# vkit-dev/vkit-ocr-model-adaptive-scaling

Hardware: AMD Instinct MI355X
Metric: images/sec fwd+bwd @1024x1024 bf16 (train step: rough+precise passes, losses, backward, clip, AdamW) (higher is better)
Workload: dtype bf16

## Files before the change

include/vkas.h:

```cpp
#ifndef VKAS_H
#define VKAS_H

#include <stddef.h>
#include <stdint.h>

#ifdef __cplusplus
extern "C" {
#endif

#define VKAS_F32 0
#define VKAS_BF16 1
#define VKAS_F16 2

#define VKAS_OK 0
#define VKAS_E_ARG (-1)
#define VKAS_E_LAUNCH (-2)

#define VKAS_EPI_NONE 0
#define VKAS_EPI_GELU 1
#define VKAS_EPI_SCALE_RES 2
#define VKAS_EPI_DGELU 3
#define VKAS_EPI_ADD 4
#define VKAS_EPI_PATCH 5
#define VKAS_EPI_HEAD 6
// ... 115 lines not shown
size_t vkas_layernorm_bwd_ws_bytes(long M, int Cp);

int vkas_pack_head_params(const float* gamma, const float* beta, const float* wproj, const float* bproj, int C, int oc,
                          int pw, float* out, void* stream);
int vkas_head_tail_fwd(const void* z, long ldz, const vkas_head_desc* hd, long M, int dtype, void* stream);
int vkas_head_tail_bwd(const void* z, long ldz, const vkas_head_desc* hd, const float* const* dproj, void* dz, long lddz,
                       float* dparams, float* ws, size_t ws_bytes, long M, int dtype, void* stream);
size_t vkas_head_tail_bwd_ws_bytes(long M, int pw);

int vkas_scale_res_bwd(const void* dout, long lddo, const void* z, long ldz, const float* colscale,
                       const float* rowscale, int rows_per_image, void* dz, long lddz, float* dscale, float* dbias,
                       float* ws, size_t ws_bytes, long M, int Cp, int dtype, void* stream);
size_t vkas_scale_res_bwd_ws_bytes(long M, int Cp);

int vkas_resize_fwd(const void* x, long ldx, void* y, long ldy, int B, int Hin, int Win, int Hout, int Wout,
                    int Cp, int mode, int accumulate, int dtype, void* stream);
int vkas_resize_bwd(const void* dy, long lddy, void* dx, long lddx, int B, int Hin, int Win, int Hout, int Wout,
                    int Cp, int mode, int accumulate, int dtype, void* stream);
size_t vkas_resize_bwd_ws_bytes(int B, int Hin, int Win, int Hout, int Wout, int Cp);
int vkas_resize_bwd_ws(const void* dy, long lddy, void* dx, long lddx, float* ws, size_t ws_bytes, int B, int Hin, int Win,
                       int Hout, int Wout, int Cp, int mode, int accumulate, int dtype, void* stream);

int vkas_upconv_adj(const void* dz, long lddz, void* E, int B, int h, int w, int N, int dtype, void* stream);
int vkas_upconv_adj_unpack_wgrad(const float* gE, float* gwp, int N, int Cp, void* stream);

int vkas_adaptive_avgpool_fwd(const void* x, long ldx, void* y, long ldy, int B, int H, int W, int s, int Cp,
                              int dtype, void* stream);
int vkas_adaptive_avgpool_bwd(const void* dy, long lddy, void* dx, long lddx, int B, int H, int W, int s, int Cp,
                              int accumulate, int dtype, void* stream);

int vkas_copy_channels(const void* x, long ldx, void* y, long ldy, long M, int Cp, int accumulate, int dtype,
                       void* stream);
int vkas_copy_channel_range(const void* x, long ldx, int c_src, void* y, long ldy, int c_dst, long M, int C,
                            int zero_tail, int dtype, void* stream);
int vkas_softplus_fwd(const float* x, float* y, long n, void* stream);
int vkas_softplus_bwd(const float* x, const float* dy, float* dx, long n, void* stream);

typedef struct vkas_rough_loss_cfg {
  float focal_factor, dice_factor, l1_factor, score_min, height_min;
  float focal_alpha, focal_gamma;
  float out_scale;
} vkas_rough_loss_cfg;
int vkas_rough_loss_fwd(const float* mask_feat, const float* height_feat, const float* gt_mask,
                        const float* gt_score, int B, int H, int W, int up, int left, int CH, int CW,
                        const vkas_rough_loss_cfg* cfg, double* sums, float* loss, void* stream);
int vkas_rough_loss_bwd(const float* mask_feat, const float* height_feat, const float* gt_mask,
// ... 42 lines not shown
#define VKAS_LOSS_FOCAL 0
#define VKAS_LOSS_DICE 1
#define VKAS_LOSS_L1 2
#define VKAS_LOSS_SMOOTH_L1 3
#define VKAS_LOSS_L2 4
#define VKAS_LOSS_WAHR 5
int vkas_elementwise_loss_fwd(int kind, const float* pred, const float* gt, const float* mask, long n, float p0, float p1,
                              float eps, double* sums, float* loss, void* stream);
int vkas_elementwise_loss_bwd(int kind, const float* pred, const float* gt, const float* mask, long n, float p0, float p1,
                              float eps, const double* sums, const float* dloss, float* dpred, void* stream);
int vkas_cross_entropy_fwd(const float* logits, const void* target, int hard, long rows, int classes, double* sums,
                           float* loss, void* stream);
int vkas_cross_entropy_bwd(const float* logits, const void* target, int hard, long rows, int classes, const float* dloss,
                           float* dlogits, void* stream);

int vkas_points_prepare(const long* py, const long* px, int B, int P, int H, int W, int* map, int* pix, long Mp, void* stream);
int vkas_points_gather_rows(const void* z, long ldz, int c0, int Ns, const float* stats, const float* const* dproj,
                            int n_heads, long M, const int* pix, long Mp, void* zs, float* stats_s, float* dproj_s,
                            int dtype, void* stream);
int vkas_points_gather_patches(const void* x, long ldx, int Cp, int B, int H, int W, const int* pix, long Mp, void* xs,
                               int dtype, void* stream);
int vkas_points_scatter3x3(const float* D, const int* pix, const int* map, long Mp, int B, int H, int W, int Cp, void* dx,
                           long lddx, int dtype, void* stream);

int vkas_points_scatter_vec8(const float* src, const int* pix, long Mp, float* dst, void* stream);
int vkas_points_gather_vec8(const float* src, const int* pix, long Mp, float* dst, void* stream);

typedef struct {
  const float* w;
  void* out;
  long total;
  int kind, N, C, KH, KW, Np, Cp, mode, n_off, Nt, dtype;
} vkas_pack_desc;
int vkas_pack_many(const vkas_pack_desc* descs, const int* block_start, int count, int total_blocks, void* stream);
int vkas_pack_many_blocks(const vkas_pack_desc* d);

int vkas_rough_postprocess(const float* mask_logit, const float* height, int B, int H, int W, const int* valid_h,
                           const int* valid_w, float mask_thr, float height_min, unsigned char* out_mask,
                           float* out_height, void* stream);
int vkas_precise_postprocess(const float* prob_logit, const float* offset, const float* angle, const float* dist, int B,
                             int H, int W, const int* valid_h, const int* valid_w, float* out_prob, float* out_offset,
                             float* out_angle, float* out_dist, void* stream);
long vkas_char_polygons_workspace_bytes(int B, int H, int W, int size);
int vkas_char_polygons(const float* prob, const float* offset, const float* angle, const float* dist, int B, int H, int W,
                       int size, float thr, float scale_y, float scale_x, void* workspace, size_t workspace_bytes,
                       int* count, int* points, float* probs, float* quads, void* stream);
// ... 20 lines not shown
```

vkit_ocr_model_adaptive_scaling_amd/_lib.py:

```python
import ctypes
import os
from ctypes import POINTER, Structure, c_char, c_char_p, c_double, c_float, c_int, c_int64, c_long, c_longlong, c_size_t, c_uint, c_void_p

_HERE = os.path.dirname(os.path.abspath(__file__))
LIB_PATH = os.environ.get('VKAS_LIB_PATH') or os.path.join(_HERE, 'libvkas.so')

F32, BF16, F16 = 0, 1, 2
EPI_NONE, EPI_GELU, EPI_SCALE_RES, EPI_DGELU, EPI_ADD, EPI_PATCH, EPI_HEAD = range(7)
LOSS_FOCAL, LOSS_DICE, LOSS_L1, LOSS_SMOOTH_L1, LOSS_L2 = range(5)
LOSS_WAHR = 5
PRECISE_LOSS_EX_SUMS = 16


class ConvGeom(Structure):
    _fields_ = [('B', c_int), ('Hin', c_int), ('Win', c_int), ('Hout', c_int), ('Wout', c_int), ('Cp', c_int),
                ('ldx', c_int), ('KH', c_int), ('KW', c_int), ('stride', c_int), ('pad', c_int)]


class HeadDesc(Structure):
    _fields_ = [('n_heads', c_int), ('pw', c_int), ('n0', c_int * 4), ('np', c_int * 4), ('c', c_int * 4),
                ('oc', c_int * 4), ('params', c_void_p), ('stats', c_void_p), ('proj', c_void_p)]


class Epilogue(Structure):
# ... 94 lines not shown
                                    POINTER(GemmPlanInfo)]),
    'vkas_colsum': (c_int, [_P, c_long, c_long, c_int, _P, c_int, _P, c_size_t, c_int, _P]),
    'vkas_colsum_ws_bytes': (c_size_t, [c_long, c_int]),
    'vkas_dwconv7x7_fwd': (c_int, [_P, c_long, _P, _P, _P, c_long, _P, c_long, c_int, c_int, c_int, c_int, c_int, _P]),
    'vkas_dwconv7x7_wgrad': (c_int, [_P, c_long, _P, c_long, _P, _P, _P, c_size_t, c_int, c_int, c_int, c_int, c_int, _P]),
    'vkas_dwconv7x7_wgrad_ws_bytes': (c_size_t, [c_int, c_int, c_int, c_int]),
    'vkas_layernorm_fwd': (c_int, [_P, c_long, _P, _P, _P, c_long, _P, c_long, c_int, c_int, c_int, c_int, _P]),
    'vkas_layernorm_bwd': (c_int, [_P, c_long, _P, _P, _P, _P, c_long, _P, c_long, _P, _P, _P, c_size_t, c_long, c_int,
                                   c_int, c_int, c_int, _P]),
    'vkas_layernorm_bwd_ws_bytes': (c_size_t, [c_long, c_int]),
    'vkas_pack_head_params': (c_int, [_P, _P, _P, _P, c_int, c_int, c_int, _P, _P]),
    'vkas_head_tail_fwd': (c_int, [_P, c_long, _P, c_long, c_int, _P]),
    'vkas_head_tail_bwd': (c_int, [_P, c_long, POINTER(HeadDesc), POINTER(c_void_p), _P, c_long, _P, _P, c_size_t, c_long, c_int, _P]),
    'vkas_head_tail_bwd_ws_bytes': (c_size_t, [c_long, c_int]),
    'vkas_scale_res_bwd': (c_int, [_P, c_long, _P, c_long, _P, _P, c_int, _P, c_long, _P, _P, _P, c_size_t, c_long,
                                   c_int, c_int, _P]),
    'vkas_scale_res_bwd_ws_bytes': (c_size_t, [c_long, c_int]),
    'vkas_resize_fwd': (c_int, [_P, c_long, _P, c_long, c_int, c_int, c_int, c_int, c_int, c_int, c_int, c_int, c_int, _P]),
    'vkas_resize_bwd': (c_int, [_P, c_long, _P, c_long, c_int, c_int, c_int, c_int, c_int, c_int, c_int, c_int, c_int, _P]),
    'vkas_resize_bwd_ws_bytes': (c_size_t, [c_int, c_int, c_int, c_int, c_int, c_int]),
    'vkas_resize_bwd_ws': (c_int, [_P, c_long, _P, c_long, _P, c_size_t, c_int, c_int, c_int, c_int, c_int, c_int, c_int, c_int,
                                   c_int, _P]),
    'vkas_upconv_adj': (c_int, [_P, c_long, _P, c_int, c_int, c_int, c_int, c_int, _P]),
    'vkas_upconv_adj_unpack_wgrad': (c_int, [_P, _P, c_int, c_int, _P]),
    'vkas_adaptive_avgpool_fwd':(c_int, [_P, c_long, _P, c_long, c_int, c_int, c_int, c_int, c_int, c_int, _P]),
    'vkas_adaptive_avgpool_bwd': (c_int, [_P, c_long, _P, c_long, c_int, c_int, c_int, c_int, c_int, c_int, c_int, _P]),
    'vkas_copy_channels': (c_int, [_P, c_long, _P, c_long, c_long, c_int, c_int, c_int, _P]),
    'vkas_copy_channel_range': (c_int, [_P, c_long, c_int, _P, c_long, c_int, c_long, c_int, c_int, c_int, _P]),
    'vkas_softplus_fwd': (c_int, [_P, _P, c_long, _P]),
    'vkas_softplus_bwd': (c_int, [_P, _P, _P, c_long, _P]),
    'vkas_rough_loss_fwd': (c_int, [_P, _P, _P, _P, c_int, c_int, c_int, c_int, c_int, c_int, c_int,
                                    POINTER(RoughLossCfg), _P, _P, _P]),
    'vkas_rough_loss_bwd': (c_int, [_P, _P, _P, _P, c_int, c_int, c_int, c_int, c_int, c_int, c_int,
                                    POINTER(RoughLossCfg), _P, _P, _P, _P, _P]),
    'vkas_points_margin': (c_int, [_P, _P, c_long, c_int, c_int, _P, _P]),
    'vkas_precise_loss_fwd': (c_int, [_P] * 11 + [c_int] * 8 + [POINTER(PreciseLossCfg), _P, _P, _P]),
    'vkas_precise_loss_bwd': (c_int, [_P] * 11 + [c_int] * 8 + [POINTER(PreciseLossCfg), _P, _P, _P, _P, _P, _P, _P]),
    'vkas_precise_loss_ex_fwd': (c_int, [_P] * 11 + [c_int] * 8 + [POINTER(PreciseLossCfg), _P, POINTER(PreciseLossExtraCfg),
                                                                     _P, _P, _P]),
    'vkas_precise_loss_ex_bwd': (c_int, [_P] * 11 + [c_int] * 8 + [POINTER(PreciseLossCfg), _P, POINTER(PreciseLossExtraCfg)]
                                 + [_P] * 8),
    'vkas_elementwise_loss_fwd': (c_int, [c_int, _P, _P, _P, c_long, c_float, c_float, c_float, _P, _P, _P]),
    'vkas_elementwise_loss_bwd': (c_int, [c_int, _P, _P, _P, c_long, c_float, c_float, c_float, _P, _P, _P, _P]),
    'vkas_cross_entropy_fwd': (c_int, [_P, _P, c_int, c_long, c_int, _P, _P, _P]),
    'vkas_cross_entropy_bwd': (c_int, [_P, _P, c_int, c_long, c_int, _P, _P, _P]),
    'vkas_points_prepare': (c_int, [_P, _P, c_int, c_int, c_int, c_int, _P, _P, c_long, _P]),
    'vkas_points_gather_rows': (c_int, [_P, c_long, c_int, c_int, _P, _P, c_int, c_long, _P, c_long, _P, _P, _P, c_int, _P]),
    'vkas_points_gather_patches': (c_int, [_P, c_long, c_int, c_int, c_int, c_int, _P, c_long, _P, c_int, _P]),
    'vkas_points_scatter3x3': (c_int, [_P, _P, _P, c_long, c_int, c_int, c_int, c_int, _P, c_long, c_int, _P]),
    'vkas_points_scatter_vec8': (c_int, [_P, _P, c_long, _P, _P]),
    'vkas_points_gather_vec8': (c_int, [_P, _P, c_long, _P, _P]),
    'vkas_pack_many': (c_int, [_P, _P, c_int, c_int, _P]),
    'vkas_pack_many_blocks': (c_int, [_P]),
    'vkas_rough_postprocess': (c_int, [_P, _P, c_int, c_int, c_int, _P, _P, c_float, c_float, _P, _P, _P]),
    'vkas_precise_postprocess': (c_int, [_P, _P, _P, _P, c_int, c_int, c_int, _P, _P, _P, _P, _P, _P, _P]),
    'vkas_char_polygons_workspace_bytes': (c_long, [c_int, c_int, c_int, c_int]),
    'vkas_char_polygons': (c_int, [_P, _P, _P, _P, c_int, c_int, c_int, c_int, c_float, c_float, c_float, _P, c_size_t,
                                   _P, _P, _P, _P, _P]),
    'vkas_text_regions_workspace_bytes': (c_longlong, [c_int, c_int, c_int, c_int]),
    'vkas_text_regions': (c_int, [_P, _P, c_int, c_int, c_int, c_int, _P, c_longlong, _P, _P, _P, _P, _P, _P, _P]),
    'vkas_resample_pack_u8': (c_int, [_P, c_int, c_int, _P, c_int, _P, c_int, c_int, _P]),
    'vkas_pack_region_labels': (c_int, [_P, c_int, c_int, c_int, c_int, c_int, c_int, _P, _P, c_int, c_int, _P, c_int, c_int,
                                        _P]),
    'vkas_l2norm_sq': (c_int, [_P, c_long, _P, _P]),
    'vkas_adamw_step': (c_int, [_P, _P, _P, _P, c_long, _P, c_float, c_float, c_float, c_float, c_float, c_float,
                                c_float, c_int, _P]),
}

EXPORTS = tuple(_SIGS)

for _name, (_res, _args) in _SIGS.items():
    _fn = getattr(lib, _name)
# ... 9 lines not shown
```

vkit_ocr_model_adaptive_scaling_amd/csrc/points.hip:

```cpp
#include "vkas_common.h"

namespace {

constexpr int PT_EMPTY = 0x7f7f7f7f;
constexpr int PT_PAD = INT_MIN;

__device__ __forceinline__ long pt_clamp(long v, int n) { return v < 0 ? 0 : (v > n - 1 ? n - 1 : v); }

__global__ __launch_bounds__(256) void points_claim_kernel(const long* __restrict__ py, const long* __restrict__ px, int P,
                                                           int H, int W, long n, int* __restrict__ map) {
  const long i = (long)blockIdx.x * 256 + threadIdx.x;
  if (i >= n) return;
  const long q = (i / P) * H * W + pt_clamp(py[i], H) * W + pt_clamp(px[i], W);
  atomicMin(&map[q], (int)i);
}

__global__ __launch_bounds__(256) void points_pix_kernel(const long* __restrict__ py, const long* __restrict__ px, int P, int H,
                                                         int W, long n, long Mp, const int* __restrict__ map,
                                                         int* __restrict__ pix) {
  const long i = (long)blockIdx.x * 256 + threadIdx.x;
  if (i >= Mp) return;
  if (i >= n) {
    pix[i] = PT_PAD;
    return;
// ... 78 lines not shown
    src[u] = o;
    if (o != PT_EMPTY && first) {
      first = false;
      mine = (o == (int)i && u == t);
    }
  }
  if (!mine) return;
  T* out = dx + (img + (long)ty * W + tx) * lddx;
  for (int v = threadIdx.x; v < (Cp >> 3); v += 64) {
    float acc[8];
    load8(out + v * 8, acc);
#pragma unroll
    for (int u = 0; u < 9; ++u) {
      if (src[u] == PT_EMPTY) continue;
      const float4* r = reinterpret_cast<const float4*>(D + ((long)src[u] * 9 + u) * Cp + v * 8);
      const float4 r0 = r[0], r1 = r[1];
      acc[0] += r0.x; acc[1] += r0.y; acc[2] += r0.z; acc[3] += r0.w;
      acc[4] += r1.x; acc[5] += r1.y; acc[6] += r1.z; acc[7] += r1.w;
    }
    store8(out + v * 8, acc);
  }
}

__global__ __launch_bounds__(256) void points_scatter_vec8_kernel(const float* __restrict__ src, const int* __restrict__ pix,
                                                                  long Mp, float* __restrict__ dst) {
  const long t = (long)blockIdx.x * 256 + threadIdx.x;
  const long i = t >> 1;
  if (i >= Mp) return;
  const int p = pix[i];
  if (p < 0) return;
  reinterpret_cast<float4*>(dst + (long)p * 8)[t & 1] = reinterpret_cast<const float4*>(src + i * 8)[t & 1];
}

__global__ __launch_bounds__(256) void points_gather_vec8_kernel(const float* __restrict__ src, const int* __restrict__ pix,
                                                                 long Mp, float* __restrict__ dst) {
  const long t = (long)blockIdx.x * 256 + threadIdx.x;
  const long i = t >> 1;
  if (i >= Mp) return;
  const int p = pix[i];
  float4 v = make_float4(0.f, 0.f, 0.f, 0.f);
  if (p >= 0) v = reinterpret_cast<const float4*>(src + (long)p * 8)[t & 1];
  reinterpret_cast<float4*>(dst + i * 8)[t & 1] = v;
}

}

// ... 58 lines not shown
                 vkas_aligned16(xs),
             "vkas_points_gather_patches: bad sizes Cp=%d ldx=%ld", Cp, ldx);
  hipStream_t st = vkas_stream(stream);
  VKAS_DISPATCH_DTYPE(dtype, "vkas_points_gather_patches", {
    points_gather_patches_kernel<T><<<(unsigned)Mp, 64, 0, st>>>((const T*)x, ldx, Cp, H, W, pix, (T*)xs);
  })
  VKAS_LAUNCH_CHECK("points_gather_patches");
  return VKAS_OK;
}

extern "C" int vkas_points_scatter3x3(const float* D, const int* pix, const int* map, long Mp, int B, int H, int W, int Cp,
                                      void* dx, long lddx, int dtype, void* stream) {
  VKAS_CHECK(D && pix && map && dx, "vkas_points_scatter3x3: null pointer");
  VKAS_CHECK(Cp > 0 && Cp % 8 == 0 && lddx >= Cp && lddx % 8 == 0 && B > 0 && H > 0 && W > 0 && Mp > 0 && Mp * 9 < 0x7fffffffL &&
                 vkas_aligned16(D) && vkas_aligned16(dx),
             "vkas_points_scatter3x3: bad sizes Cp=%d lddx=%ld Mp=%ld", Cp, lddx, Mp);
  hipStream_t st = vkas_stream(stream);
  VKAS_DISPATCH_DTYPE(dtype, "vkas_points_scatter3x3", {
    points_scatter3x3_kernel<T><<<(unsigned)(Mp * 9), 64, 0, st>>>(D, pix, map, H, W, Cp, (T*)dx, lddx);
  })
  VKAS_LAUNCH_CHECK("points_scatter3x3");
  return VKAS_OK;
}
```

vkit_ocr_model_adaptive_scaling_amd/csrc/upconv_adj.hip:

```cpp
#include "vkas_common.h"

namespace {

__device__ __forceinline__ int xcd_row(unsigned bx, unsigned rows) {
  const unsigned xcd = bx & 7u, slot = bx >> 3;
  const unsigned q8 = rows >> 3, r8 = rows & 7u;
  return (int)((xcd < r8 ? xcd * (q8 + 1) : r8 * (q8 + 1) + (xcd - r8) * q8) + slot);
}

__device__ __forceinline__ void ut_weights(int i, int n, float* w) {
  w[0] = i == 0 ? 0.f : 0.25f;
  w[1] = i == 0 ? 1.f : 0.75f;
  w[2] = i == n - 1 ? 1.f : 0.75f;
  w[3] = i == n - 1 ? 0.f : 0.25f;
}

template <typename T>
__global__ __launch_bounds__(256) void upconv_adj_kernel(const T* __restrict__ dz, long lddz, T* __restrict__ E, int h,
                                                         int w, int nvec) {
  const int idx = blockIdx.y * 256 + threadIdx.x;
  const int j = idx / nvec;
  const int v = idx - j * nvec;
  if (j >= w) return;
  const int row = xcd_row(blockIdx.x, gridDim.x);
  const int b = row / h;
  const int i = row - b * h;
  const int H2 = 2 * h, W2 = 2 * w;
  float wy[4], wx[4];
  ut_weights(i, h, wy);
  ut_weights(j, w, wx);
  int xc[6];
  bool xok[6];
#pragma unroll
  for (int c = 0; c < 6; ++c) {
    const int X = 2 * j - 2 + c;
    xok[c] = X >= 0 && X < W2;
    xc[c] = X < 0 ? 0 : (X >= W2 ? W2 - 1 : X);
  }
  const T* db = dz + (long)b * H2 * W2 * lddz + v * 8;
  float acc[3][3][8];
#pragma unroll
  for (int ky = 0; ky < 3; ++ky)
#pragma unroll
    for (int kx = 0; kx < 3; ++kx)
#pragma unroll
      for (int k = 0; k < 8; ++k) acc[ky][kx][k] = 0.f;
#pragma unroll
  for (int r = 0; r < 6; ++r) {
    const int Y = 2 * i - 2 + r;
    const bool yok = Y >= 0 && Y < H2;
    const int yc = Y < 0 ? 0 : (Y >= H2 ? H2 - 1 : Y);
    const T* rowp = db + (long)yc * W2 * lddz;
    Raw8<T> raw[6];
#pragma unroll
    for (int c = 0; c < 6; ++c) raw[c].load(rowp + (long)xc[c] * lddz);
    float hs[3][8];
#pragma unroll
    for (int kx = 0; kx < 3; ++kx)
#pragma unroll
      for (int k = 0; k < 8; ++k) hs[kx][k] = 0.f;
#pragma unroll
    for (int c = 0; c < 6; ++c) {
      raw[c].keep_if(yok && xok[c]);
      float t[8];
      raw[c].unpack(t);
#pragma unroll
      for (int kx = 0; kx < 3; ++kx) {
        const int a = c - kx;
        if (a < 0 || a > 3) continue;
#pragma unroll
        for (int k = 0; k < 8; ++k) hs[kx][k] = fmaf(wx[a], t[k], hs[kx][k]);
      }
    }
#pragma unroll
    for (int ky = 0; ky < 3; ++ky) {
      const int a = r - ky;
      if (a < 0 || a > 3) continue;
#pragma unroll
      for (int kx = 0; kx < 3; ++kx)
#pragma unroll
        for (int k = 0; k < 8; ++k) acc[ky][kx][k] = fmaf(wy[a], hs[kx][k], acc[ky][kx][k]);
    }
  }
  const long N = (long)nvec * 8;
  T* dst = E + (((long)b * h + i) * w + j) * (9 * N) + v * 8;
#pragma unroll
  for (int ky = 0; ky < 3; ++ky)
#pragma unroll
    for (int kx = 0; kx < 3; ++kx) store8(dst + (ky * 3 + kx) * N, acc[ky][kx]);
}

__global__ __launch_bounds__(256) void upconv_adj_unpack_kernel(const float* __restrict__ gE, float* __restrict__ gwp, int N,
                                                                int Cp4, long total4) {
  for (long i = (long)blockIdx.x * 256 + threadIdx.x; i < total4; i += (long)gridDim.x * 256) {
    const int c4 = (int)(i % Cp4);
    const long r = i / Cp4;
    const int n = (int)(r % N);
    const int k = (int)(r / N);
    const float4 s = reinterpret_cast<const float4*>(gE)[i];
    float4* d = reinterpret_cast<float4*>(gwp) + ((long)n * 9 + (8 - k)) * Cp4 + c4;
    float4 o = *d;
    o.x += s.x; o.y += s.y; o.z += s.z; o.w += s.w;
    *d = o;
  }
}

}

extern "C" int vkas_upconv_adj(const void* dz, long lddz, void* E, int B, int h, int w, int N, int dtype, void* stream) {
  VKAS_CHECK(dz && E && vkas_aligned16(dz) && vkas_aligned16(E), "vkas_upconv_adj: null/misaligned tensor");
  VKAS_CHECK(B >= 0 && h > 0 && w > 0, "vkas_upconv_adj: bad spatial dims");
  VKAS_CHECK(N > 0 && N % 8 == 0 && lddz >= N && lddz % 8 == 0, "vkas_upconv_adj: bad channels/stride (N=%d lddz=%ld)", N, lddz);
  VKAS_CHECK(dtype == VKAS_BF16 || dtype == VKAS_F16, "vkas_upconv_adj: 16-bit storage only");
  if (B == 0) return VKAS_OK;
  VKAS_CHECK((long)B * h < (1L << 31) && (long)w * (N / 8) < (1L << 30) && vkas_cdiv((long)w * (N / 8), 256) <= 65535,
             "vkas_upconv_adj: map too large");
  dim3 grid((unsigned)((long)B * h), (unsigned)vkas_cdiv((long)w * (N / 8), 256));
  if (dtype == VKAS_BF16)
    upconv_adj_kernel<bf16_t><<<grid, 256, 0, vkas_stream(stream)>>>((const bf16_t*)dz, lddz, (bf16_t*)E, h, w, N / 8);
  else
    upconv_adj_kernel<f16_t><<<grid, 256, 0, vkas_stream(stream)>>>((const f16_t*)dz, lddz, (f16_t*)E, h, w, N / 8);
  VKAS_LAUNCH_CHECK("upconv_adj");
  return VKAS_OK;
}

extern "C" int vkas_upconv_adj_unpack_wgrad(const float* gE, float* gwp, int N, int Cp, void* stream) {
  VKAS_CHECK(gE && gwp && vkas_aligned16(gE) && vkas_aligned16(gwp), "vkas_upconv_adj_unpack_wgrad: null/misaligned pointer");
  VKAS_CHECK(N > 0 && Cp > 0 && Cp % 8 == 0, "vkas_upconv_adj_unpack_wgrad: bad sizes (N=%d Cp=%d)", N, Cp);
  const long total4 = 9L * N * (Cp / 4);
  long g = vkas_cdiv(total4, 256);
  if (g > 4096) g = 4096;
  upconv_adj_unpack_kernel<<<(unsigned)g, 256, 0, vkas_stream(stream)>>>(gE, gwp, N, Cp / 4, total4);
  VKAS_LAUNCH_CHECK("upconv_adj_unpack_wgrad");
  return VKAS_OK;
}
```

vkit_ocr_model_adaptive_scaling_amd/ops.py:

```python
import copy
import ctypes
import os
import weakref
from typing import Optional, Sequence, Tuple

import torch
from torch.autograd import Function

from . import _lib
from ._lib import lib, check, ConvGeom, Epilogue

_FLOAT = torch.float32


def rup8(c: int) -> int:
    return (c + 7) // 8 * 8


_DTYPE_CODES = {torch.float32: _lib.F32, torch.bfloat16: _lib.BF16, torch.float16: _lib.F16}
_MFMA_DTYPES = (torch.bfloat16, torch.float16)


def _dtc(dtype: torch.dtype) -> int:
    try:
# ... 951 lines not shown


def _heads_dense_upres(heads, r0, r1, pw, hp, x, z, stats, dps, dparams, gwp, gbp, dx_up):
    B, H, W, Cp = x.shape
    offs, K, C = heads.offs, 9 * Cp, heads.C
    Nd = offs[r1] - offs[r0]
    dz = _heads_dense_dz(heads, r0, r1, pw, hp, x, z, stats, dps, dparams)
    geom = _geom(B, H, W, H, W, Cp, act_ld(x), 3, 3, 1, 1)
    conv_wgrad(x, geom, dz, Nd, nk=(sum(heads.cs[r0:r1]), C * 9), with_bias=True,
               gw_into=gwp[offs[r0] * K:offs[r1] * K], gb_into=gbp[offs[r0]:offs[r1]])
    if dx_up is not None:
        Bt = heads.weights(1, x.dtype, r0, r1)
        g2 = _geom(B, H, W, H, W, Nd, Nd, 3, 3, 1, 1)
        conv_gemm(dz, g2, Bt, Cp, dx_up, _lib.EPI_NONE, nk=(C, sum(heads.cs[r0:r1]) * 9))


def _heads_dense_lowres(heads, r0, r1, pw, hp, x, z, stats, dps, dparams, gwp, gbp, x_low, dx):
    B, H, W, Cp = x.shape
    h_, w_, M = H // 2, W // 2, B * H * W
    offs, K, C, es = heads.offs, 9 * Cp, heads.C, x.element_size()
    Nd = offs[r1] - offs[r0]
    dz = _heads_dense_dz(heads, r0, r1, pw, hp, x, z, stats, dps, dparams)
    E = new_act(B, h_, w_, 9 * Nd, x)
    _timed('upconv_adj_kernel', x, 0.0, M // 4, 9 * Nd, 0,
           lambda: check(lib.vkas_upconv_adj(_p(dz), act_ld(dz), _p(E), B, h_, w_, Nd, _dt(x), _stream()), 'upconv_adj'),
           float(M) * Nd * es * 3.25)
    nbytes = lib.vkas_colsum_ws_bytes(M, Nd)
    ws_cs = _ws(nbytes, x.device)
    _timed('colsum_partial_kernel', x, 0.0, M, Nd, 0,
           lambda: check(lib.vkas_colsum(_p(dz), act_ld(dz), M, Nd, _p(gbp[offs[r0]:offs[r1]]), 1, _p(ws_cs), nbytes,
                                         _dt(x), _stream()), 'colsum'), float(M) * Nd * es)
    del dz
    g1 = _geom(B, h_, w_, h_, w_, Cp, act_ld(x_low), 1, 1, 1, 0)
    gE = conv_wgrad(x_low, g1, E, 9 * Nd, nk=(9 * sum(heads.cs[r0:r1]), C), step_scratch=True)
    check(lib.vkas_upconv_adj_unpack_wgrad(_p(gE), _p(gwp[offs[r0] * K:offs[r1] * K]), Nd, Cp, _stream()),
          'upconv_adj_unpack_wgrad')
    if dx is not None:
        Bt = heads.weights(1, x.dtype, r0, r1)
        g2 = _geom(B, h_, w_, h_, w_, 9 * Nd, 9 * Nd, 1, 1, 1, 0)
        conv_gemm(E, g2, Bt, Cp, dx, _lib.EPI_NONE, nk=(C, sum(heads.cs[r0:r1]) * 9))


def _heads_points_grads(heads, h0, h1, pw, hp, patches, zs, stats_s, dp_ptrs, pix, pmap, n_points, dparams, gw_into, gb_into,
                        step_scratch, dx_into):
    Mp, Ns, K, C = zs.shape[2], zs.shape[3], 9 * heads.Cp, heads.C
    dzs = new_act(1, 1, Mp, Ns, zs)
    _head_tail_bwd(heads, h0, h1, pw, hp, zs.data_ptr(), Ns, stats_s.data_ptr(), dp_ptrs, Mp, dzs, dparams)
    xs = patches() if callable(patches) else patches
    g1 = _geom(1, 1, Mp, 1, Mp, K, K, 1, 1, 1, 0)
    gw, gb = conv_wgrad(xs, g1, dzs, Ns, nk=(sum(heads.cs[h0:h1]), C * 9), with_bias=True, gw_into=gw_into, gb_into=gb_into,
                        step_scratch=step_scratch)
    if dx_into is not None:
        B, H, W, Cp = dx_into.shape
        Wf = heads.weights(0, zs.dtype)[heads.offs[h0] * K:heads.offs[h1] * K].view(1, 1, Ns, K)
        dzt = dzs.view(Mp, Ns).t().contiguous().view(1, 1, Ns, Mp)
        g3 = _geom(1, 1, Ns, 1, Ns, K, K, 1, 1, 1, 0)
        D = conv_wgrad(Wf, g3, dzt, Mp, nk=(n_points, C * 9), step_scratch=True, ordered=True)
        check(lib.vkas_points_scatter3x3(_p(D), _p(pix), _p(pmap), Mp, B, H, W, Cp, _p(dx_into), act_ld(dx_into), _dt(zs),
                                         _stream()), 'points_scatter3x3')
    return gw, gb


def _deliver_head_weight_grads(heads, gwp, K):
    gws = []
    for h in range(heads.n):
        sw = grad_sink(heads.ws[h])
        g = unpack_wgrad(gwp[heads.offs[h] * K:heads.offs[h + 1] * K], (heads.cs[h], heads.C, 3, 3), heads.nps[h], heads.Cp,
                         into=heads.ws[h].grad if sw is not None else None)
        if sw is not None:
            sw[0].grad_delivered(sw[1])
        gws.append(None if sw is not None else g)
    return gws


def _deliver_head_small_grads(heads, pw, dparams, gbp, flat_sinks):
    outs, pieces, delivered = [], [], []
    for h in range(heads.n):
        c, oc = heads.cs[h], heads.ocs[h]
        out, views = [], heads.small_grad_views(h, pw, dparams[h], gbp)
        for j, (param, g) in enumerate(zip((heads.bs[h], heads.gammas[h], heads.betas[h], heads.wps[h], heads.bps[h]), views)):
            sk = grad_sink(param)
            if sk is None or not param.grad.is_contiguous():
# ... 55 lines not shown
        ctx.heads, ctx.pw, ctx.low = heads, pw, x_low is not None
        return tuple(proj[h] for h in range(n_heads))

    @staticmethod
    def backward(ctx, *dprojs):
        saved = ctx.saved_tensors
        x, z, stats, hp = saved[:4]
        pw, n_heads = ctx.pw, ctx.heads.n
        heads = ctx.heads.from_saved(saved[4:4 + 6 * n_heads])
        B, H, W, Cp = x.shape
        Nt, M, K, dev = heads.Nt, B * H * W, 9 * Cp, x.device
        dparams = torch.empty((n_heads, 6 * pw + 8), dtype=_FLOAT, device=dev)
        flat_sinks = all(grad_sink(p) is not None for p in list(heads.ws) + list(heads.bs))
        gbuf = zeros_f32(Nt * K + Nt, dev, flat_sinks)
        gwp, gbp = gbuf[:Nt * K], gbuf[Nt * K:]
        dps = [torch.zeros((B, H, W, 8), dtype=_FLOAT, device=dev) if dp is None else dp.contiguous().float() for dp in dprojs]
        sp = _point_sparse_run(dprojs, B, H, W) if _POINT_SPARSE else None
        low, h_, w_ = ctx.low, H // 2, W // 2
        x_low = saved[4 + 6 * n_heads] if low else None
        (s0, s1), (u0, u1), (e0, e1) = _head_bwd_plan(n_heads, sp and sp[:2], [point_mark(d) is not None for d in dprojs], low)
        need_dx = ctx.needs_input_grad[0]
        dx = (new_act(B, h_, w_, Cp, x) if low else new_act(B, H, W, Cp, x)) if need_dx else None
        dx_pts = dx
        if low and need_dx and u1 == u0:
            dx_pts = torch.zeros((B, H, W, Cp), dtype=x.dtype, device=dev) if sp is not None else None
        elif low:
            dx_pts = new_act(B, H, W, Cp, x) if need_dx else None
        elif u1 == u0 and dx is not None:
            dx.zero_()
        if u1 > u0:
            _heads_dense_upres(heads, u0, u1, pw, hp, x, z, stats, dps, dparams, gwp, gbp, dx_pts)
        if e1 > e0:
            _heads_dense_lowres(heads, e0, e1, pw, hp, x, z, stats, dps, dparams, gwp, gbp, x_low, dx)
        if sp is not None:
            offs, Ns, py, px = heads.offs, heads.offs[s1] - heads.offs[s0], sp[2], sp[3]
            _, pmap, pix, Mp = _points_prepare(py, px, B, H, W)
            zs = new_act(1, 1, Mp, Ns, x)
            fbuf = torch.empty(((s1 - s0) * Mp * 10,), dtype=_FLOAT, device=dev)
            stats_s, dproj_s = fbuf[:(s1 - s0) * Mp * 2], fbuf[(s1 - s0) * Mp * 2:]
            ptrs = (ctypes.c_void_p * 4)(*[dps[h].data_ptr() for h in range(s0, s1)])
            check(lib.vkas_points_gather_rows(_p(z), Nt, offs[s0], Ns, ctypes.c_void_p(stats.data_ptr() + s0 * M * 8), ptrs,
                                              s1 - s0, M, _p(pix), Mp, _p(zs), _p(stats_s), _p(dproj_s), _dt(x), _stream()),
                  'points_gather_rows')
            _heads_points_grads(heads, s0, s1, pw, hp, lambda: _points_gather_patches(x, pix, Mp), zs, stats_s,
                                [dproj_s.data_ptr() + j * Mp * 32 for j in range(s1 - s0)], pix, pmap, py.numel(), dparams,
                                gwp[offs[s0] * K:offs[s1] * K], gbp[offs[s0]:offs[s1]], False, dx_pts)
        if low and dx is not None:
            if dx_pts is not None:
                _timed('resize2x_bwd_kernel', x, 0.0, M, Cp, 0,
                       lambda: check(lib.vkas_resize_bwd(_p(dx_pts), act_ld(dx_pts), _p(dx), act_ld(dx), B, h_, w_, H, W, Cp, 0,
                                                         int(e1 > e0), _dt(x), _stream()), 'resize_bwd'),
                       B * Cp * x.element_size() * (h_ * w_ * (2 if e1 > e0 else 1) + H * W))
            elif e1 == e0:
                dx.zero_()
        gws = _deliver_head_weight_grads(heads, gwp, K)
        small = _deliver_head_small_grads(heads, pw, dparams, gbp, flat_sinks)
        return (dx, None, *[g for h in range(n_heads) for g in (gws[h], *small[h])])


_HEAD_BWD_UPRES = os.environ.get('VKAS_HEAD_BWD_UPRES') is not None


class UpHeadsFused(Function):

    @staticmethod
    def eligible(x, channels, out_channels) -> bool:
        B, h, w, _ = x.shape
        return not _HEAD_BWD_UPRES and h > 1 and w > 1 and _heads_eligible(x.dtype, 4 * B * h * w, channels, out_channels)

    @staticmethod
# ... 65 lines not shown
        saved = ctx.saved_tensors
        xs, zs, stats_s, hp, scratch = saved[:5]
        heads = ctx.heads.from_saved(saved[5:])
        n_heads, M, K, dev = heads.n, B * H * W, 9 * Cp, xs.device
        pmap, pix = scratch[:M], scratch[M:]
        dproj_s = torch.empty((n_heads, Mp, 8), dtype=_FLOAT, device=dev)
        for h in range(n_heads):
            if dprojs[h] is None:
                dproj_s[h].zero_()
            else:
                check(lib.vkas_points_gather_vec8(_p(dprojs[h].contiguous().float()), _p(pix), Mp, _p(dproj_s[h]), _stream()),
                      'points_gather_vec8')
        dparams = torch.empty((n_heads, 6 * pw + 8), dtype=_FLOAT, device=dev)
        dx = torch.zeros((B, H, W, Cp), dtype=dtype, device=dev) if ctx.needs_input_grad[0] else None
        flat_sinks = all(grad_sink(p) is not None for p in list(heads.ws) + list(heads.bs))
        gwp, gbp = _heads_points_grads(heads, 0, n_heads, pw, hp, xs, zs, stats_s, [d.data_ptr() for d in dproj_s], pix, pmap,
                                       B * P, dparams, None, None, flat_sinks, dx)
        gws = _deliver_head_weight_grads(heads, gwp, K)
        grads = [g for h in range(n_heads) for g in (gws[h], *heads.small_grad_views(h, pw, dparams[h], gbp))]
        return (dx, None, None, *grads)


_POINT_SPARSE = os.environ.get('VKAS_POINT_SPARSE_BWD', '1') != '0'


def point_sparse(grad: torch.Tensor, py: torch.Tensor, px: torch.Tensor) -> torch.Tensor:
    grad._vkas_points = (py, px, grad._version)
    return grad


def point_mark(t: Optional[torch.Tensor]):
    m = getattr(t, '_vkas_points', None) if t is not None else None
    if m is None or t._version != m[2]:
        return None
    return m[0], m[1]


def pass_point_sparse(src: torch.Tensor, dst: torch.Tensor) -> torch.Tensor:
    pts = point_mark(src)
    if pts is not None:
        point_sparse(dst, pts[0], pts[1])
    return dst


def _point_sparse_run(dprojs, B, H, W):
    marks = [point_mark(d) for d in dprojs]
# ... 847 lines not shown
```

Baseline: 269.1.

## Fuse bias colsum into upconv adjoint and scatter point grads directly at low resolution

The dense head backward now computes the bias column-sum inside the upconv adjoint kernel, so the separate colsum pass no longer re-reads dz. The point-sparse head backward now scatters 3x3 gradients straight into the low-resolution dx by folding in the 2x upsample adjoint weights. This skips allocating and zeroing a full-resolution dx buffer and skips the resize backward pass. In exchange the kernels are more complex: the colsum kernel uses shared-memory reduction with a workspace plus a finalize step, and the low scatter kernel needs per-block ownership checks over a 6x6 neighbourhood.

Result: faster. 274.0 (median of 6 runs) (+1.8%).

```diff
diff --git a/include/vkas.h b/include/vkas.h
--- a/include/vkas.h
+++ b/include/vkas.h
@@ -161,6 +161,9 @@
                        int Hout, int Wout, int Cp, int mode, int accumulate, int dtype, void* stream);
 
 int vkas_upconv_adj(const void* dz, long lddz, void* E, int B, int h, int w, int N, int dtype, void* stream);
+size_t vkas_upconv_adj_colsum_ws_bytes(int B, int h, int w, int N);
+int vkas_upconv_adj_colsum(const void* dz, long lddz, void* E, int B, int h, int w, int N, float* out, int accumulate, float* ws,
+                           size_t ws_bytes, int dtype, void* stream);
 int vkas_upconv_adj_unpack_wgrad(const float* gE, float* gwp, int N, int Cp, void* stream);
 
 int vkas_adaptive_avgpool_fwd(const void* x, long ldx, void* y, long ldy, int B, int H, int W, int s, int Cp,
@@ -249,6 +252,8 @@
                                int dtype, void* stream);
 int vkas_points_scatter3x3(const float* D, const int* pix, const int* map, long Mp, int B, int H, int W, int Cp, void* dx,
                            long lddx, int dtype, void* stream);
+int vkas_points_scatter3x3_low(const float* D, const int* pix, const int* map, long Mp, int B, int h, int w, int Cp, void* dx,
+                               long lddx, int dtype, void* stream);
 
 int vkas_points_scatter_vec8(const float* src, const int* pix, long Mp, float* dst, void* stream);
 int vkas_points_gather_vec8(const float* src, const int* pix, long Mp, float* dst, void* stream);
diff --git a/profiles/kernel_table.py b/profiles/kernel_table.py
--- /dev/null
+++ b/profiles/kernel_table.py
@@ -0,0 +1,36 @@
+#!/usr/bin/env python3
+import collections
+import csv
+import re
+import sys
+
+
+def short(name):
+    name = re.sub(r'^_ZN12_GLOBAL__N_1\d+', '', name)
+    f = re.search(r'FillFunctor<([^>]*)>', name)
+    if f:
+        return 'aten_fill<%s>' % f.group(1)
+    m = re.search(r'(\w+_kernel|\w+Functor<[^>]*>|__amd_\w+)', name)
+    return m.group(1) if m else name[:60]
+
+
+def main():
+    want = sys.argv[2:]
+    rows = collections.OrderedDict()
+    with open(sys.argv[1], newline='') as f:
+        for r in csv.DictReader(f):
+            name = short(r['Kernel_Name'])
+            if want and not any(w in name for w in want):
+                continue
+            key = (name, int(r['Grid_Size_X']), int(r['Grid_Size_Y']), int(r['Workgroup_Size_X']))
+            d = rows.setdefault(key, [0, 0])
+            d[0] += 1
+            d[1] += int(r['End_Timestamp']) - int(r['Start_Timestamp'])
+    out = csv.writer(sys.stdout)
+    out.writerow(['kernel', 'grid_x', 'grid_y', 'workgroup', 'calls', 'total_us', 'mean_us'])
+    for (name, gx, gy, wg), (n, ns) in sorted(rows.items(), key=lambda kv: -kv[1][1]):
+        out.writerow([name, gx, gy, wg, n, '%.1f' % (ns / 1e3), '%.1f' % (ns / 1e3 / n)])
+
+
+if __name__ == '__main__':
+    main()
diff --git a/profiles/peak_memory.py b/profiles/peak_memory.py
--- /dev/null
+++ b/profiles/peak_memory.py
@@ -0,0 +1,16 @@
+#!/usr/bin/env python3
+import json
+import os
+import sys
+
+ROOT = os.path.dirname(os.path.dirname(os.path.abspath(__file__)))
+sys.path.insert(0, ROOT)
+import torch
+import bench
+
+if __name__ == '__main__':
+    sys.argv = [os.path.join(ROOT, 'bench.py')] + (sys.argv[1:] or ['--gpus', '1', '--steps', '3', '--warmup', '2'])
+    bench.main()
+    torch.cuda.synchronize()
+    print(json.dumps({'max_memory_allocated_MiB': round(torch.cuda.max_memory_allocated() / 2**20, 1),
+                      'max_memory_reserved_MiB': round(torch.cuda.max_memory_reserved() / 2**20, 1)}))
diff --git a/vkit_ocr_model_adaptive_scaling_amd/_lib.py b/vkit_ocr_model_adaptive_scaling_amd/_lib.py
--- a/vkit_ocr_model_adaptive_scaling_amd/_lib.py
+++ b/vkit_ocr_model_adaptive_scaling_amd/_lib.py
@@ -140,6 +140,8 @@
     'vkas_resize_bwd_ws': (c_int, [_P, c_long, _P, c_long, _P, c_size_t, c_int, c_int, c_int, c_int, c_int, c_int, c_int, c_int,
                                    c_int, _P]),
     'vkas_upconv_adj': (c_int, [_P, c_long, _P, c_int, c_int, c_int, c_int, c_int, _P]),
+    'vkas_upconv_adj_colsum_ws_bytes': (c_size_t, [c_int, c_int, c_int, c_int]),
+    'vkas_upconv_adj_colsum': (c_int, [_P, c_long, _P, c_int, c_int, c_int, c_int, _P, c_int, _P, c_size_t, c_int, _P]),
     'vkas_upconv_adj_unpack_wgrad': (c_int, [_P, _P, c_int, c_int, _P]),
     'vkas_adaptive_avgpool_fwd':(c_int, [_P, c_long, _P, c_long, c_int, c_int, c_int, c_int, c_int, c_int, _P]),
     'vkas_adaptive_avgpool_bwd': (c_int, [_P, c_long, _P, c_long, c_int, c_int, c_int, c_int, c_int, c_int, c_int, _P]),
@@ -166,6 +168,7 @@
     'vkas_points_gather_rows': (c_int, [_P, c_long, c_int, c_int, _P, _P, c_int, c_long, _P, c_long, _P, _P, _P, c_int, _P]),
     'vkas_points_gather_patches': (c_int, [_P, c_long, c_int, c_int, c_int, c_int, _P, c_long, _P, c_int, _P]),
     'vkas_points_scatter3x3': (c_int, [_P, _P, _P, c_long, c_int, c_int, c_int, c_int, _P, c_long, c_int, _P]),
+    'vkas_points_scatter3x3_low': (c_int, [_P, _P, _P, c_long, c_int, c_int, c_int, c_int, _P, c_long, c_int, _P]),
     'vkas_points_scatter_vec8': (c_int, [_P, _P, c_long, _P, _P]),
     'vkas_points_gather_vec8': (c_int, [_P, _P, c_long, _P, _P]),
     'vkas_pack_many': (c_int, [_P, _P, c_int, c_int, _P]),
diff --git a/vkit_ocr_model_adaptive_scaling_amd/csrc/points.hip b/vkit_ocr_model_adaptive_scaling_amd/csrc/points.hip
--- a/vkit_ocr_model_adaptive_scaling_amd/csrc/points.hip
+++ b/vkit_ocr_model_adaptive_scaling_amd/csrc/points.hip
@@ -124,6 +124,77 @@
   }
 }
 
+__device__ __forceinline__ void pt_ut_weights(int i, int n, float* w) {
+  w[0] = i == 0 ? 0.f : 0.25f;
+  w[1] = i == 0 ? 1.f : 0.75f;
+  w[2] = i == n - 1 ? 1.f : 0.75f;
+  w[3] = i == n - 1 ? 0.f : 0.25f;
+}
+
+template <typename T>
+__global__ __launch_bounds__(64) void points_scatter3x3_low_kernel(const float* __restrict__ D, const int* __restrict__ pix,
+                                                                   const int* __restrict__ map, int h, int w, int Cp,
+                                                                   T* __restrict__ dx, long lddx) {
+  const long i = blockIdx.x / 9;
+  const int t = (int)(blockIdx.x - i * 9);
+  const int p = pix[i];
+  if (p < 0) return;
+  const int H = 2 * h, W = 2 * w;
+  const long q = p;
+  const int xx = (int)(q % W), yy = (int)((q / W) % H);
+  const long img = q - ((long)yy * W + xx);
+  const int si = (yy >> 1) + t / 3 - 1, sj = (xx >> 1) + t % 3 - 1;
+  if ((unsigned)si >= (unsigned)h || (unsigned)sj >= (unsigned)w) return;
+  int src[36];
+  bool first = true, mine = false;
+#pragma unroll
+  for (int e = 0; e < 36; ++e) {
+    const int Y = 2 * si - 2 + e / 6, X = 2 * sj - 2 + e % 6;
+    const bool ok = (unsigned)Y < (unsigned)H && (unsigned)X < (unsigned)W;
+    const int yc = Y < 0 ? 0 : (Y > H - 1 ? H - 1 : Y), xc = X < 0 ? 0 : (X > W - 1 ? W - 1 : X);
+    int o = map[img + (long)yc * W + xc];
+    o = __builtin_amdgcn_readfirstlane(ok ? o : PT_EMPTY);
+    src[e] = o;
+    if (o != PT_EMPTY && first) {
+      first = false;
+      mine = o == (int)i;
+    }
+  }
+  if (!mine) return;
+  float wy[4], wx[4];
+  pt_ut_weights(si, h, wy);
+  pt_ut_weights(sj, w, wx);
+  const int nv = Cp >> 3;
+  T* out = dx + ((img >> 2) + (long)si * w + sj) * lddx;
+  for (int v0 = 0; v0 < nv; v0 += 64) {
+    const int v = v0 + (int)threadIdx.x;
+    const int vc = v < nv ? v : nv - 1;
+    float old[8], acc[8];
+    load8(out + vc * 8, old);
+#pragma unroll
+    for (int k = 0; k < 8; ++k) acc[k] = 0.f;
+#pragma unroll
+    for (int e = 0; e < 36; ++e) {
+      if (src[e] == PT_EMPTY) continue;
+      const float* Dp = D + (long)src[e] * 9 * Cp + vc * 8;
+#pragma unroll
+      for (int u = 0; u < 9; ++u) {
+        const int a = e / 6 + u / 3 - 2, c = e % 6 + u % 3 - 2;
+        if (a < 0 || a > 3 || c < 0 || c > 3) continue;
+        const float wq = wy[a] * wx[c];
+        const float4* r = reinterpret_cast<const float4*>(Dp + (long)u * Cp);
+        const float4 r0 = r[0], r1 = r[1];
+        acc[0] = fmaf(wq, r0.x, acc[0]); acc[1] = fmaf(wq, r0.y, acc[1]); acc[2] = fmaf(wq, r0.z, acc[2]);
+        acc[3] = fmaf(wq, r0.w, acc[3]); acc[4] = fmaf(wq, r1.x, acc[4]); acc[5] = fmaf(wq, r1.y, acc[5]);
+        acc[6] = fmaf(wq, r1.z, acc[6]); acc[7] = fmaf(wq, r1.w, acc[7]);
+      }
+    }
+#pragma unroll
+    for (int k = 0; k < 8; ++k) old[k] += acc[k];
+    if (v < nv) store8(out + v * 8, old);
+  }
+}
+
 __global__ __launch_bounds__(256) void points_scatter_vec8_kernel(const float* __restrict__ src, const int* __restrict__ pix,
                                                                   long Mp, float* __restrict__ dst) {
   const long t = (long)blockIdx.x * 256 + threadIdx.x;
@@ -228,3 +299,17 @@
   VKAS_LAUNCH_CHECK("points_scatter3x3");
   return VKAS_OK;
 }
+
+extern "C" int vkas_points_scatter3x3_low(const float* D, const int* pix, const int* map, long Mp, int B, int h, int w, int Cp,
+                                          void* dx, long lddx, int dtype, void* stream) {
+  VKAS_CHECK(D && pix && map && dx, "vkas_points_scatter3x3_low: null pointer");
+  VKAS_CHECK(Cp > 0 && Cp % 8 == 0 && lddx >= Cp && lddx % 8 == 0 && B > 0 && h > 0 && w > 0 && Mp > 0 && Mp * 9 < 0x7fffffffL &&
+                 4L * B * h * w < PT_EMPTY && vkas_aligned16(D) && vkas_aligned16(dx),
+             "vkas_points_scatter3x3_low: bad sizes Cp=%d lddx=%ld Mp=%ld", Cp, lddx, Mp);
+  hipStream_t st = vkas_stream(stream);
+  VKAS_DISPATCH_DTYPE(dtype, "vkas_points_scatter3x3_low", {
+    points_scatter3x3_low_kernel<T><<<(unsigned)(Mp * 9), 64, 0, st>>>(D, pix, map, h, w, Cp, (T*)dx, lddx);
+  })
+  VKAS_LAUNCH_CHECK("points_scatter3x3_low");
+  return VKAS_OK;
+}
diff --git a/vkit_ocr_model_adaptive_scaling_amd/csrc/upconv_adj.hip b/vkit_ocr_model_adaptive_scaling_amd/csrc/upconv_adj.hip
--- a/vkit_ocr_model_adaptive_scaling_amd/csrc/upconv_adj.hip
+++ b/vkit_ocr_model_adaptive_scaling_amd/csrc/upconv_adj.hip
@@ -1,4 +1,6 @@
 #include "vkas_common.h"
+
+int vkas_colreduce_finalize(const float* partial, long P, int n, int ldp, float* out, int accumulate, hipStream_t st);
 
 namespace {
 
@@ -13,6 +15,84 @@
   w[1] = i == 0 ? 1.f : 0.75f;
   w[2] = i == n - 1 ? 1.f : 0.75f;
   w[3] = i == n - 1 ? 0.f : 0.25f;
+}
+
+template <typename T, bool CS>
+__device__ __forceinline__ void upconv_adj_pair(const T* __restrict__ dz, long lddz, T* __restrict__ E, int h, int w, int nvec,
+                                                int b, int i, int j, int v, float* cs) {
+  const int H2 = 2 * h, W2 = 2 * w;
+  float wy[4], wx[4];
+  ut_weights(i, h, wy);
+  ut_weights(j, w, wx);
+  int xc[6];
+  bool xok[6];
+#pragma unroll
+  for (int c = 0; c < 6; ++c) {
+    const int X = 2 * j - 2 + c;
+    xok[c] = X >= 0 && X < W2;
+    xc[c] = X < 0 ? 0 : (X >= W2 ? W2 - 1 : X);
+  }
+  const T* db = dz + (long)b * H2 * W2 * lddz + v * 8;
+  float acc[3][3][8];
+#pragma unroll
+  for (int ky = 0; ky < 3; ++ky)
+#pragma unroll
+    for (int kx = 0; kx < 3; ++kx)
+#pragma unroll
+      for (int k = 0; k < 8; ++k) acc[ky][kx][k] = 0.f;
+#pragma unroll
+  for (int r = 0; r < 6; ++r) {
+    const int Y = 2 * i - 2 + r;
+    const bool yok = Y >= 0 && Y < H2;
+    const int yc = Y < 0 ? 0 : (Y >= H2 ? H2 - 1 : Y);
+    Raw8<T> raw[6];
+    if constexpr (CS) {
+      const T* rowb = dz + ((long)b * H2 + yc) * W2 * lddz;
+#pragma unroll
+      for (int c = 0; c < 6; ++c) raw[c].load(rowb + (unsigned)(xc[c] * (int)lddz + v * 8));
+    } else {
+      const T* rowp = db + (long)yc * W2 * lddz;
+#pragma unroll
+      for (int c = 0; c < 6; ++c) raw[c].load(rowp + (long)xc[c] * lddz);
+    }
+    float hs[3][8];
+#pragma unroll
+    for (int kx = 0; kx < 3; ++kx)
+#pragma unroll
+      for (int k = 0; k < 8; ++k) hs[kx][k] = 0.f;
+#pragma unroll
+    for (int c = 0; c < 6; ++c) {
+      raw[c].keep_if(yok && xok[c]);
+      float t[8];
+      raw[c].unpack(t);
+      if (CS && (r == 2 || r == 3) && (c == 2 || c == 3)) {
+#pragma unroll
+        for (int k = 0; k < 8; ++k) cs[k * 256] += t[k];
+      }
+#pragma unroll
+      for (int kx = 0; kx < 3; ++kx) {
+        const int a = c - kx;
+        if (a < 0 || a > 3) continue;
+#pragma unroll
+        for (int k = 0; k < 8; ++k) hs[kx][k] = fmaf(wx[a], t[k], hs[kx][k]);
+      }
+    }
+#pragma unroll
+    for (int ky = 0; ky < 3; ++ky) {
+      const int a = r - ky;
+      if (a < 0 || a > 3) continue;
+#pragma unroll
+      for (int kx = 0; kx < 3; ++kx)
+#pragma unroll
+        for (int k = 0; k < 8; ++k) acc[ky][kx][k] = fmaf(wy[a], hs[kx][k], acc[ky][kx][k]);
+    }
+  }
+  const long N = (long)nvec * 8;
+  T* dst = E + (((long)b * h + i) * w + j) * (9 * N) + v * 8;
+#pragma unroll
+  for (int ky = 0; ky < 3; ++ky)
+#pragma unroll
+    for (int kx = 0; kx < 3; ++kx) store8(dst + (ky * 3 + kx) * N, acc[ky][kx]);
 }
 
 template <typename T>
@@ -24,70 +104,35 @@
   if (j >= w) return;
   const int row = xcd_row(blockIdx.x, gridDim.x);
   const int b = row / h;
+  upconv_adj_pair<T, false>(dz, lddz, E, h, w, nvec, b, row - b * h, j, v, nullptr);
+}
+
+template <typename T>
+__global__ __launch_bounds__(256, 2) void upconv_adj_colsum_kernel(const T* __restrict__ dz, long lddz, T* __restrict__ E, int h,
+                                                                int w, int nvec, float* __restrict__ partial) {
+  const int ppc = 256 / nvec;
+  const int jl = threadIdx.x / nvec;
+  const int v = threadIdx.x - jl * nvec;
+  const int row = xcd_row(blockIdx.x, gridDim.x);
+  const int b = __builtin_amdgcn_readfirstlane(row / h);
   const int i = row - b * h;
-  const int H2 = 2 * h, W2 = 2 * w;
-  float wy[4], wx[4];
-  ut_weights(i, h, wy);
-  ut_weights(j, w, wx);
-  int xc[6];
-  bool xok[6];
-#pragma unroll
-  for (int c = 0; c < 6; ++c) {
-    const int X = 2 * j - 2 + c;
-    xok[c] = X >= 0 && X < W2;
-    xc[c] = X < 0 ? 0 : (X >= W2 ? W2 - 1 : X);
-  }
-  const T* db = dz + (long)b * H2 * W2 * lddz + v * 8;
-  float acc[3][3][8];
-#pragma unroll
-  for (int ky = 0; ky < 3; ++ky)
-#pragma unroll
-    for (int kx = 0; kx < 3; ++kx)
-#pragma unroll
-      for (int k = 0; k < 8; ++k) acc[ky][kx][k] = 0.f;
-#pragma unroll
-  for (int r = 0; r < 6; ++r) {
-    const int Y = 2 * i - 2 + r;
-    const bool yok = Y >= 0 && Y < H2;
-    const int yc = Y < 0 ? 0 : (Y >= H2 ? H2 - 1 : Y);
-    const T* rowp = db + (long)yc * W2 * lddz;
-    Raw8<T> raw[6];
-#pragma unroll
-    for (int c = 0; c < 6; ++c) raw[c].load(rowp + (long)xc[c] * lddz);
-    float hs[3][8];
-#pragma unroll
-    for (int kx = 0; kx < 3; ++kx)
-#pragma unroll
-      for (int k = 0; k < 8; ++k) hs[kx][k] = 0.f;
-#pragma unroll
-    for (int c = 0; c < 6; ++c) {
-      raw[c].keep_if(yok && xok[c]);
-      float t[8];
-      raw[c].unpack(t);
-#pragma unroll
-      for (int kx = 0; kx < 3; ++kx) {
-        const int a = c - kx;
-        if (a < 0 || a > 3) continue;
-#pragma unroll
-        for (int k = 0; k < 8; ++k) hs[kx][k] = fmaf(wx[a], t[k], hs[kx][k]);
-      }
-    }
-#pragma unroll
-    for (int ky = 0; ky < 3; ++ky) {
-      const int a = r - ky;
-      if (a < 0 || a > 3) continue;
-#pragma unroll
-      for (int kx = 0; kx < 3; ++kx)
-#pragma unroll
-        for (int k = 0; k < 8; ++k) acc[ky][kx][k] = fmaf(wy[a], hs[kx][k], acc[ky][kx][k]);
-    }
-  }
-  const long N = (long)nvec * 8;
-  T* dst = E + (((long)b * h + i) * w + j) * (9 * N) + v * 8;
-#pragma unroll
-  for (int ky = 0; ky < 3; ++ky)
-#pragma unroll
-    for (int kx = 0; kx < 3; ++kx) store8(dst + (ky * 3 + kx) * N, acc[ky][kx]);
+  __shared__ float red[8 * 256];
+#pragma unroll
+  for (int k = 0; k < 8; ++k) red[k * 256 + threadIdx.x] = 0.f;
+  if (jl < ppc) {
+    for (int j = blockIdx.y * ppc + jl; j < w; j += gridDim.y * ppc)
+      upconv_adj_pair<T, true>(dz, lddz, E, h, w, nvec, b, i, j, v, red + threadIdx.x);
+  }
+  __syncthreads();
+  if (jl == 0) {
+    float cs[8];
+#pragma unroll
+    for (int k = 0; k < 8; ++k) cs[k] = red[k * 256 + v];
+    for (int r = 1; r < ppc; ++r)
+#pragma unroll
+      for (int k = 0; k < 8; ++k) cs[k] += red[k * 256 + r * nvec + v];
+    store8(partial + ((long)blockIdx.x * gridDim.y + blockIdx.y) * ((long)nvec * 8) + v * 8, cs);
+  }
 }
 
 __global__ __launch_bounds__(256) void upconv_adj_unpack_kernel(const float* __restrict__ gE, float* __restrict__ gwp, int N,
@@ -124,6 +169,41 @@
   return VKAS_OK;
 }
 
+namespace {
+static inline long cs_groups(int B, int h, int w, int N) {
+  const long chunks = vkas_cdiv(w, 256 / (N / 8));
+  long g = 4096 / ((long)B * h);
+  g = g < 1 ? 1 : g;
+  return g < chunks ? g : chunks;
+}
+}
+
+extern "C" size_t vkas_upconv_adj_colsum_ws_bytes(int B, int h, int w, int N) {
+  if (B <= 0 || h <= 0 || w <= 0 || N <= 0 || N % 8 || N > 2048) return 0;
+  return (size_t)B * h * cs_groups(B, h, w, N) * N * sizeof(float);
+}
+
+extern "C" int vkas_upconv_adj_colsum(const void* dz, long lddz, void* E, int B, int h, int w, int N, float* out, int accumulate,
+                                      float* ws, size_t ws_bytes, int dtype, void* stream) {
+  VKAS_CHECK(dz && E && out && ws && vkas_aligned16(dz) && vkas_aligned16(E) && vkas_aligned16(ws),
+             "vkas_upconv_adj_colsum: null/misaligned pointer");
+  VKAS_CHECK(B > 0 && h > 0 && w > 0 && (long)B * h < (1L << 31) && 2L * w * lddz < (1L << 31),
+             "vkas_upconv_adj_colsum: bad spatial dims");
+  VKAS_CHECK(N > 0 && N % 8 == 0 && N <= 2048 && lddz >= N && lddz % 8 == 0,
+             "vkas_upconv_adj_colsum: bad channels/stride (N=%d lddz=%ld)", N, lddz);
+  VKAS_CHECK(dtype == VKAS_BF16 || dtype == VKAS_F16, "vkas_upconv_adj_colsum: 16-bit storage only");
+  VKAS_CHECK(ws_bytes >= vkas_upconv_adj_colsum_ws_bytes(B, h, w, N), "vkas_upconv_adj_colsum: workspace too small");
+  const long G = cs_groups(B, h, w, N);
+  dim3 grid((unsigned)((long)B * h), (unsigned)G);
+  hipStream_t st = vkas_stream(stream);
+  if (dtype == VKAS_BF16)
+    upconv_adj_colsum_kernel<bf16_t><<<grid, 256, 0, st>>>((const bf16_t*)dz, lddz, (bf16_t*)E, h, w, N / 8, ws);
+  else
+    upconv_adj_colsum_kernel<f16_t><<<grid, 256, 0, st>>>((const f16_t*)dz, lddz, (f16_t*)E, h, w, N / 8, ws);
+  VKAS_LAUNCH_CHECK("upconv_adj_colsum");
+  return vkas_colreduce_finalize(ws, (long)B * h * G, N, N, out, accumulate, st);
+}
+
 extern "C" int vkas_upconv_adj_unpack_wgrad(const float* gE, float* gwp, int N, int Cp, void* stream) {
   VKAS_CHECK(gE && gwp && vkas_aligned16(gE) && vkas_aligned16(gwp), "vkas_upconv_adj_unpack_wgrad: null/misaligned pointer");
   VKAS_CHECK(N > 0 && Cp > 0 && Cp % 8 == 0, "vkas_upconv_adj_unpack_wgrad: bad sizes (N=%d Cp=%d)", N, Cp);
diff --git a/vkit_ocr_model_adaptive_scaling_amd/ops.py b/vkit_ocr_model_adaptive_scaling_amd/ops.py
--- a/vkit_ocr_model_adaptive_scaling_amd/ops.py
+++ b/vkit_ocr_model_adaptive_scaling_amd/ops.py
@@ -997,14 +997,12 @@
     Nd = offs[r1] - offs[r0]
     dz = _heads_dense_dz(heads, r0, r1, pw, hp, x, z, stats, dps, dparams)
     E = new_act(B, h_, w_, 9 * Nd, x)
-    _timed('upconv_adj_kernel', x, 0.0, M // 4, 9 * Nd, 0,
-           lambda: check(lib.vkas_upconv_adj(_p(dz), act_ld(dz), _p(E), B, h_, w_, Nd, _dt(x), _stream()), 'upconv_adj'),
+    nbytes = lib.vkas_upconv_adj_colsum_ws_bytes(B, h_, w_, Nd)
+    ws_cs = _ws(nbytes, x.device)
+    _timed('upconv_adj_colsum_kernel', x, 0.0, M // 4, 9 * Nd, 0,
+           lambda: check(lib.vkas_upconv_adj_colsum(_p(dz), act_ld(dz), _p(E), B, h_, w_, Nd, _p(gbp[offs[r0]:offs[r1]]), 1,
+                                                    _p(ws_cs), nbytes, _dt(x), _stream()), 'upconv_adj_colsum'),
            float(M) * Nd * es * 3.25)
-    nbytes = lib.vkas_colsum_ws_bytes(M, Nd)
-    ws_cs = _ws(nbytes, x.device)
-    _timed('colsum_partial_kernel', x, 0.0, M, Nd, 0,
-           lambda: check(lib.vkas_colsum(_p(dz), act_ld(dz), M, Nd, _p(gbp[offs[r0]:offs[r1]]), 1, _p(ws_cs), nbytes,
-                                         _dt(x), _stream()), 'colsum'), float(M) * Nd * es)
     del dz
     g1 = _geom(B, h_, w_, h_, w_, Cp, act_ld(x_low), 1, 1, 1, 0)
     gE = conv_wgrad(x_low, g1, E, 9 * Nd, nk=(9 * sum(heads.cs[r0:r1]), C), step_scratch=True)
@@ -1017,7 +1015,7 @@
 
 
 def _heads_points_grads(heads, h0, h1, pw, hp, patches, zs, stats_s, dp_ptrs, pix, pmap, n_points, dparams, gw_into, gb_into,
-                        step_scratch, dx_into):
+                        step_scratch, dx_into, dx_low=False):
     Mp, Ns, K, C = zs.shape[2], zs.shape[3], 9 * heads.Cp, heads.C
     dzs = new_act(1, 1, Mp, Ns, zs)
     _head_tail_bwd(heads, h0, h1, pw, hp, zs.data_ptr(), Ns, stats_s.data_ptr(), dp_ptrs, Mp, dzs, dparams)
@@ -1031,8 +1029,12 @@
         dzt = dzs.view(Mp, Ns).t().contiguous().view(1, 1, Ns, Mp)
         g3 = _geom(1, 1, Ns, 1, Ns, K, K, 1, 1, 1, 0)
         D = conv_wgrad(Wf, g3, dzt, Mp, nk=(n_points, C * 9), step_scratch=True, ordered=True)
-        check(lib.vkas_points_scatter3x3(_p(D), _p(pix), _p(pmap), Mp, B, H, W, Cp, _p(dx_into), act_ld(dx_into), _dt(zs),
-                                         _stream()), 'points_scatter3x3')
+        if dx_low:
+            check(lib.vkas_points_scatter3x3_low(_p(D), _p(pix), _p(pmap), Mp, B, H, W, Cp, _p(dx_into), act_ld(dx_into),
+                                                 _dt(zs), _stream()), 'points_scatter3x3_low')
+        else:
+            check(lib.vkas_points_scatter3x3(_p(D), _p(pix), _p(pmap), Mp, B, H, W, Cp, _p(dx_into), act_ld(dx_into), _dt(zs),
+                                             _stream()), 'points_scatter3x3')
     return gw, gb
 
 
@@ -1134,7 +1136,10 @@
         need_dx = ctx.needs_input_grad[0]
         dx = (new_act(B, h_, w_, Cp, x) if low else new_act(B, H, W, Cp, x)) if need_dx else None
         dx_pts = dx
-        if low and need_dx and u1 == u0:
+        pts_low = low and need_dx and u1 == u0 and sp is not None and _POINTS_LOW_SCATTER
+        if pts_low:
+            dx_pts = None
+        elif low and need_dx and u1 == u0:
             dx_pts = torch.zeros((B, H, W, Cp), dtype=x.dtype, device=dev) if sp is not None else None
         elif low:
             dx_pts = new_act(B, H, W, Cp, x) if need_dx else None
@@ -1154,10 +1159,12 @@
             check(lib.vkas_points_gather_rows(_p(z), Nt, offs[s0], Ns, ctypes.c_void_p(stats.data_ptr() + s0 * M * 8), ptrs,
                                               s1 - s0, M, _p(pix), Mp, _p(zs), _p(stats_s), _p(dproj_s), _dt(x), _stream()),
                   'points_gather_rows')
+            if pts_low and e1 == e0:
+                dx.zero_()
             _heads_points_grads(heads, s0, s1, pw, hp, lambda: _points_gather_patches(x, pix, Mp), zs, stats_s,
                                 [dproj_s.data_ptr() + j * Mp * 32 for j in range(s1 - s0)], pix, pmap, py.numel(), dparams,
-                                gwp[offs[s0] * K:offs[s1] * K], gbp[offs[s0]:offs[s1]], False, dx_pts)
-        if low and dx is not None:
+                                gwp[offs[s0] * K:offs[s1] * K], gbp[offs[s0]:offs[s1]], False, dx if pts_low else dx_pts, pts_low)
+        if low and dx is not None and not pts_low:
             if dx_pts is not None:
                 _timed('resize2x_bwd_kernel', x, 0.0, M, Cp, 0,
                        lambda: check(lib.vkas_resize_bwd(_p(dx_pts), act_ld(dx_pts), _p(dx), act_ld(dx), B, h_, w_, H, W, Cp, 0,
@@ -1269,6 +1276,7 @@
 
 
 _POINT_SPARSE = os.environ.get('VKAS_POINT_SPARSE_BWD', '1') != '0'
+_POINTS_LOW_SCATTER = os.environ.get('VKAS_POINTS_UPRES_SCATTER', '0') != '1'
 
 
 def point_sparse(grad: torch.Tensor, py: torch.Tensor, px: torch.Tensor) -> torch.Tensor:
```
